# alv-around/mini-stark

Hardware: AMD Instinct MI355X
Metric: stark_proofs_per_s (higher is better)
Workload: dtype u64; 1 GPU; Fibonacci AIR, Goldilocks, 2^20 trace rows, blowup 8, 20 security bits (w=3, c=6, rounds=23, ood_queries=1, fri_queries=2); a step = 8 independent proofs in flight per GPU

## Files before the change

mini-stark_amd/csrc/fri_commit.cpp:

```cpp
#include "ctx.hpp"
#include "digest.hpp"
#include "fri_tail.hpp"

namespace msctx {

template <class F>
int Ctx<F>::round_commit(Round* r, size_t ncoef_in, int nonzero_limbs, const Round* prev, const XE* alpha) {
  if (ctz64(r->D) > F::TWO_ADICITY) return fail(MS_ERR_SHAPE, "FRI domain larger than the field's two-adicity");
  RQ(tree_shape(r->D, 2, 2, &r->ts));
  r->m = 0;
  r->base_cw = false;
  {
    const bool shard_next = shardable(r->D / 2);
    bool z_outside_base = false;
    for (int l = 1; l < E; l++) z_outside_base = z_outside_base || cur_z.c[l] != 0;
    if (prev && fri_pointwise && z_outside_base && prev->D == 2 * r->D && prev->ts.sharded == shard_next) {
      Plan* pl;
      RQ(get_plan(ctz64(prev->D), 0, false, &pl));
      const size_t W = (size_t)sh_world;
      const size_t m_out = shard_next ? r->D / (2 * W) : r->D;
      const size_t local = shard_next ? 2 * m_out : r->D;
      if (shard_next) r->m = m_out;
      if (r->cw.ensure(local * E * sizeof(T))) return fail(MS_ERR_NOMEM, "codeword");
      const size_t total = m_out * (shard_next ? 2 : 1);
// ... 239 lines not shown
  if (next_dist) { if (nr->poly.ensure(Sn * E * sizeof(T))) return fail(MS_ERR_NOMEM, "fold"); lq = nr->poly.template as<T>(); }
  else { if (d_lq.ensure(Sn * E * sizeof(T))) return fail(MS_ERR_NOMEM, "fold"); lq = d_lq.as<T>(); }
  if (d_folded.ensure((Sn + 1) * E * sizeof(T)) || d_carry.ensure(4096)) return fail(MS_ERR_NOMEM, "fold");
  if (4 * E * sizeof(T) * (size_t)sh_world > xcap) return fail(MS_ERR_NOMEM, "exchange buffers");
  size_t nq_coef = 0;
  PartScope part(this);
  if (m >= 2) {
    T* pay = reinterpret_cast<T*>(xs);
    typename mspoly::FoldKernel<F, E>::Params fp{lpoly(pr), lstride(pr), cntp, d_folded.as<T>(), Sn, a, pay};
    if (cnt) CK(run<mspoly::FoldKernel<F, E>>(K_FOLD, grid1(cnt, mspoly::THREADS), 1, mspoly::THREADS, 0, fp));
    else CK(msrt::memset_dev(xs, 0, 2 * E * sizeof(T), stream));
    const size_t mj = cnt ? cnt - 1 : 0;
    SHPlan pl; pl.nl = 0;
    if (mj) {
      if (d_sh.ensure(sh_scratch_elems(mj) * sizeof(T))) return fail(MS_ERR_NOMEM, "scan levels");
      pl = sh_plan(d_folded.as<T>(), Sn, 1, 1, mj, cur_z, lq, false, Sn, 1, 1, nullptr, d_sh.as<T>(), d_carry.as<T>(), pay + E, true);
      for (int l = 0; l + 1 < pl.nl; l++) RQ(sh_launch_inline(pl.agg[l], 0));
      RQ(sh_launch_inline(pl.top_agg, 0));
    }
    RQ(exchange(MS_XCHG_ALL_GATHER, 2 * E * sizeof(T)));
    typedef mspoly::ShardCarryKernel<F, E> CKn;
    typename CKn::Params cp;
    memset(&cp, 0, sizeof cp);
    cp.jobs = nullptr; cp.njobs = 1; cp.W = (u32)sh_world; cp.rank = (u32)sh_rank; cp.gathered = reinterpret_cast<const T*>(xr); cp.rank_stride = 2 * E;
    cp.inline_job.first_off = 0; cp.inline_job.agg_off = E; cp.inline_job.has_first = 1;
    cp.inline_job.zA = cur_z; cp.inline_job.zB = e_pow<F, E>(cur_z, (u64)(Sn - 1));
    cp.inline_job.scale = mj ? carry_scale(cur_z, mj, pl.P) : e_one<F, E>();
    cp.inline_job.carry_out = d_carry.as<T>();
    cp.inline_job.tail_out = cnt ? lq + (cnt - 1) : nullptr; cp.inline_job.tail_stride = Sn;
    cp.inline_job.h0_out = nullptr;
    CK(run<CKn>(K_SUFFIX_HORNER, 1, 1, CKn::THREADS, 0, cp));
    if (mj) for (int l = pl.nl - 1; l >= 0; l--) RQ(sh_launch_inline(pl.fin[l], 1));
    nq_coef = m - 1;
  }
  nr->S = Sn;
  if (next_dist) { nr->dist = true; nr->local_store = true; }
  else {
    if (nr->poly.ensure(nr->cap * E * sizeof(T))) return fail(MS_ERR_NOMEM, "fold");
    if (nq_coef) RQ(gather_poly(lq, Sn, nq_coef, nr->poly.template as<T>(), nr->cap));
    nr->S = 0;
  }
  *nq_coef_out = nq_coef;
  return 0;
}

template <class F>
int Ctx<F>::fri_tail_round(Round* pr, Round* nr, const XE& a, bool* done) {
  return msmerkle::with_digest(digest, [&](auto family) { return fri_tail_round_t<decltype(family)>(pr, nr, a, done); });
}
template <class F> template <class DG>
int Ctx<F>::fri_tail_round_t(Round* pr, Round* nr, const XE& a, bool* done) {
  *done = false;
  const size_t n = pr->ncoef, m = (n + 1) / 2, Dn = nr->D, M = Dn / 2;
  bool z_outside_base = false;
  for (int l = 1; l < E; l++) z_outside_base = z_outside_base || cur_z.c[l] != 0;
  if (!fri_tail_max || pr->D > fri_tail_max || pr->dist || pr->ts.sharded || shardable(M) || !fri_pointwise || !z_outside_base || m > (size_t)mspoly::SH_BS || M < 1) return 0;
  typedef msfri::FriTailKernel<F, E, DG> TK;
  if (M > (size_t)TK::WG_GROUPS << TK::TreeK::MAX_LEVELS) return 0;
  if (ctz64(Dn) > F::TWO_ADICITY) return fail(MS_ERR_SHAPE, "FRI domain larger than the field's two-adicity");
  RQ(tree_shape(Dn, 2, 2, &nr->ts));
  nr->m = 0; nr->base_cw = false;
  if (nr->poly.ensure(nr->cap * E * sizeof(T)) || d_folded.ensure((m + 1) * E * sizeof(T)) || nr->cw.ensure(Dn * E * sizeof(T)) || nr->nodes.ensure(nr->ts.nodes * 32) ||
      d_sh.ensure(sh_scratch_elems(m) * sizeof(T)))
    return fail(MS_ERR_NOMEM, "fused FRI round");
  Plan* pl;
  RQ(get_plan(ctz64(pr->D), 0, false, &pl));
  typename TK::Params tp;
  memset(&tp, 0, sizeof tp);
  tp.do_coef = m >= 2 ? 1 : 0;
  tp.fold = typename TK::FoldK::Params{pr->poly.template as<T>(), pr->cap, n, d_folded.as<T>(), m, a, nullptr};
  if (tp.do_coef) {
    SHPlan sp = sh_plan(d_folded.as<T>(), m, 0, 1, m, cur_z, nr->poly.template as<T>(), false, nr->cap, 0, 1, nullptr, d_sh.as<T>());
    if (sp.nl != 1) return fail(MS_ERR_STATE, "fused FRI round: scan of more than one block");
    tp.scan.jobs = nullptr; tp.scan.inline_job = sp.fin[0]; tp.scan.final_mode = 1;
  }
  tp.deg = typename TK::DegK::Params{nr->poly.template as<T>(), nr->cap, m >= 2 ? m - 1 : 0, res.word(Results::FRI_LEN), 0};
  const size_t per = M < (size_t)TK::WG_GROUPS ? M : (size_t)TK::WG_GROUPS, G = M / per;
  tp.G = (u32)G;
  const XE c = e_add<F, E>(cur_B[0], e_mul<F>(cur_B[1], a));
  tp.eval.src = pr->cw.template as<T>(); tp.eval.src_limb_stride = pr->D; tp.eval.dst = nr->cw.template as<T>(); tp.eval.dst_limb_stride = Dn;
  tp.eval.m_out = Dn; tp.eval.log_m = (u32)ctz64(Dn); tp.eval.groups = 1; tp.eval.shard_W = 0; tp.eval.shard_k = 0;
  tp.eval.tw_lo = pl->tw_lo.template as<T>(); tp.eval.tw_hi = pl->tw_hi.template as<T>(); tp.eval.lo_bits = (u32)pl->lo_bits; tp.eval.log_D = (u32)ctz64(pr->D);
  tp.eval.alpha = a; tp.eval.c2 = e_add<F, E>(c, c); tp.eval.z = cur_z; tp.eval.inv2 = f_inv<F>(F::from_u64(2));
  tp.leaf.base = nr->cw.template as<T>(); tp.leaf.col_stride = 0; tp.leaf.row_stride = 1; tp.leaf.limb_stride = Dn; tp.leaf.width = 1; tp.leaf.lpn = 2;
  tp.leaf.zero_as_empty = zae; tp.leaf.ngroups = M; tp.leaf.nodes = nr->nodes.template as<u32>();
  u32 nl = 0; while (((size_t)1 << nl) < per) nl++;
  tp.sub.nodes = nr->nodes.template as<u32>(); tp.sub.child_off = 0; tp.sub.nchildren = M; tp.sub.ic = 2; tp.sub.nlevels = nl;
  u32 tl = 0; while (((size_t)1 << tl) < G) tl++;
  tp.top.nodes = nr->nodes.template as<u32>(); tp.top.child_off = 2 * M - 2 * G; tp.top.nchildren = G; tp.top.ic = 2; tp.top.nlevels = tl;
  RQ(res.attach(tp.top));
  tp.root_index = nr->ts.nodes - 1;
  tp.done = reinterpret_cast<u32*>(res.word(Results::TAIL_DONE));
  next_bytes = (double)Dn * E * sizeof(T) * 3 + (double)M * 96;
  CK(run_coop<TK>(K_FRI_TAIL, (unsigned)(G + 1), TK::THREADS, TK::lds_bytes(), tp));
  *done = true;
  return 0;
}

template <class F>
int Ctx<F>::fri_fold_commit(const u64* alpha, u8* root) {
  if (!have_deep) return fail(MS_ERR_STATE, "fri_fold_commit before fri_deep");
  XE a;
  if (!alpha || !root || !load_ext(alpha, &a)) return fail(MS_ERR_ARG, "alpha");
  Round* pr = rounds[nrounds_done - 1];
  if (pr->D < 4) return fail(MS_ERR_SHAPE, "FRI round domain too small to fold (merkle.rs:93-104 panics)");
  const size_t n = pr->ncoef, m = (n + 1) / 2;
  Round* nr = round_slot(nrounds_done);
  nr->cap = m ? m : 1;
  nr->D = pr->D / 2;
  nr->dist = false; nr->local_store = false; nr->S = 0;
  size_t nq_coef = 0;
  bool fused = false, side = false;
  unsigned long long* dres = res.word(Results::FRI_LEN), ncoef = 0;
  auto stage = res.expect(dres, pr->dist && dist_chunk(nr->D) == pr->S / 2);
  RQ(fri_tail_round(pr, nr, a, &fused));
  if (!fused) {
  if (pr->dist) RQ(fold_dist(pr, nr, a, &nq_coef));
  else {
  if (nr->poly.ensure(nr->cap * E * sizeof(T)) || d_folded.ensure((m + 1) * E * sizeof(T))) return fail(MS_ERR_NOMEM, "fold");
  if (m >= 2) {
    side = fri_overlap && !prof_on;
    if (side) RQ(res.fork_side());
    StreamScope on_side(this, side ? side_stream : stream);
    typename mspoly::FoldKernel<F, E>::Params fp{pr->poly.template as<T>(), pr->cap, n, d_folded.as<T>(), m, a, nullptr};
    CK(run<mspoly::FoldKernel<F, E>>(K_FOLD, grid1(m, mspoly::THREADS), 1, mspoly::THREADS, 0, fp));
    RQ(suffix_horner(d_folded.as<T>(), m, 0, 1, m, cur_z, nr->poly.template as<T>(), nr->cap, 0, 1, nullptr));
    nq_coef = m - 1;
  }
  }
  if (nr->dist) {
    const size_t lc = lcount(nr, nq_coef);
    if (lc) {
      typename mspoly::DegreeKernel<F, E>::Params dp{lpoly(nr), lstride(nr), lc, dres, (size_t)sh_rank * nr->S};
      PartScope part(this);
      CK(run<mspoly::DegreeKernel<F, E>>(K_DEGREE, grid1(lc, mspoly::THREADS), 1, mspoly::THREADS, 0, dp));
    }
  } else if (nq_coef) {
    StreamScope on_side(this, side ? side_stream : stream);
    typename mspoly::DegreeKernel<F, E>::Params dp{nr->poly.template as<T>(), nr->cap, nq_coef, dres, 0};
    CK(run<mspoly::DegreeKernel<F, E>>(K_DEGREE, grid1(nq_coef, mspoly::THREADS), 1, mspoly::THREADS, 0, dp));
  }
  RQ(res.side_done());
  RQ(round_commit(nr, nq_coef, E, pr, &a));
  }
  RQ(read_root(nr->nodes, nr->ts, root, &ncoef));
  nr->ncoef = (size_t)ncoef;
  nrounds_done++; have_deep = false;
  return MS_OK;
}

template <class F>
int Ctx<F>::fri_round_info(int r, u64* ncoef, u64* D) {
  if (r < 0 || (size_t)r >= nrounds_done) return fail(MS_ERR_ARG, "round index");
  if (ncoef) *ncoef = rounds[r]->ncoef;
  if (D) *D = rounds[r]->D;
  return MS_OK;
}

template <class F>
int Ctx<F>::fri_round_poly_read(int r, u64* out) {
  if (r < 0 || (size_t)r >= nrounds_done || !out) return fail(MS_ERR_ARG, "round index");
  if (rounds[r]->local_store) return fail(MS_ERR_STATE, "round_poly_read: the polynomial of a sharded round is distributed over the ranks");
  return download_widen(rounds[r]->poly.template as<T>(), rounds[r]->ncoef, rounds[r]->cap, E, out);
}

template <class F>
int Ctx<F>::fri_round_codeword_read(int r, u64* out) {
// ... 28 lines not shown
```

mini-stark_amd/csrc/merkle.hpp:

```cpp
#pragma once
#include "field.hpp"

namespace msmerkle {

constexpr int THREADS = 256;
constexpr int OVF_WORDS = 2;
constexpr int OVF_LISTS = 256;
constexpr int PAD_GRID_Y = 4;
struct alignas(16) uint4_t { u32 x, y, z, w; };

MS_HD u32 rotr32(u32 x, int n) {
#if defined(__HIP_DEVICE_COMPILE__)
  return __builtin_amdgcn_alignbit(x, x, n);
#else
  return (x >> n) | (x << (32 - n));
#endif
}
MS_HD u32 bswap32(u32 x) { return __builtin_bswap32(x); }
MS_HD u32 ch3(u32 e, u32 f, u32 g) {
#if defined(__HIP_DEVICE_COMPILE__) && __has_builtin(__builtin_amdgcn_bitop3_b32)
  return __builtin_amdgcn_bitop3_b32(e, f, g, 0xCA);
#else
  return g ^ (e & (f ^ g));
#endif
}
MS_HD u32 maj3(u32 a, u32 b, u32 c) {
#if defined(__HIP_DEVICE_COMPILE__) && __has_builtin(__builtin_amdgcn_bitop3_b32)
  return __builtin_amdgcn_bitop3_b32(a, b, c, 0xE8);
#else
  return (a & b) | (c & (a | b));
#endif
}
MS_HD u32 xor3(u32 a, u32 b, u32 c) {
#if defined(__HIP_DEVICE_COMPILE__) && __has_builtin(__builtin_amdgcn_bitop3_b32)
  return __builtin_amdgcn_bitop3_b32(a, b, c, 0x96);
#else
  return a ^ b ^ c;
#endif
}

constexpr u32 SHA_K[64] = {
    0x428a2f98, 0x71374491, 0xb5c0fbcf, 0xe9b5dba5, 0x3956c25b, 0x59f111f1, 0x923f82a4, 0xab1c5ed5,
    0xd807aa98, 0x12835b01, 0x243185be, 0x550c7dc3, 0x72be5d74, 0x80deb1fe, 0x9bdc06a7, 0xc19bf174,
    0xe49b69c1, 0xefbe4786, 0x0fc19dc6, 0x240ca1cc, 0x2de92c6f, 0x4a7484aa, 0x5cb0a9dc, 0x76f988da,
    0x983e5152, 0xa831c66d, 0xb00327c8, 0xbf597fc7, 0xc6e00bf3, 0xd5a79147, 0x06ca6351, 0x14292967,
    0x27b70a85, 0x2e1b2138, 0x4d2c6dfc, 0x53380d13, 0x650a7354, 0x766a0abb, 0x81c2c92e, 0x92722c85,
    0xa2bfe8a1, 0xa81a664b, 0xc24b8b70, 0xc76c51a3, 0xd192e819, 0xd6990624, 0xf40e3585, 0x106aa070,
    0x19a4c116, 0x1e376c08, 0x2748774c, 0x34b0bcb5, 0x391c0cb3, 0x4ed8aa4a, 0x5b9cca4f, 0x682e6ff3,
    0x748f82ee, 0x78a5636f, 0x84c87814, 0x8cc70208, 0x90befffa, 0xa4506ceb, 0xbef9a3f7, 0xc67178f2};

struct PadBlockKW { u32 kw[64]; };
constexpr u32 c_rotr(u32 x, int n) { return (x >> n) | (x << (32 - n)); }
constexpr PadBlockKW make_pad_block_kw(u32 msg_bits) {
  PadBlockKW r{};
  u32 w[64] = {};
  w[0] = 0x80000000u; w[15] = msg_bits;
  for (int i = 16; i < 64; i++) {
    const u32 s0 = c_rotr(w[i - 15], 7) ^ c_rotr(w[i - 15], 18) ^ (w[i - 15] >> 3);
    const u32 s1 = c_rotr(w[i - 2], 17) ^ c_rotr(w[i - 2], 19) ^ (w[i - 2] >> 10);
    w[i] = w[i - 16] + s0 + w[i - 7] + s1;
  }
  for (int i = 0; i < 64; i++) r.kw[i] = SHA_K[i] + w[i];
  return r;
}
template <u32 MSG_BITS> struct PadBlock { static constexpr PadBlockKW T = make_pad_block_kw(MSG_BITS); };

struct Sha256 {
  u32 st[8];
  MS_HD void init() {
    st[0] = 0x6a09e667; st[1] = 0xbb67ae85; st[2] = 0x3c6ef372; st[3] = 0xa54ff53a;
    st[4] = 0x510e527f; st[5] = 0x9b05688c; st[6] = 0x1f83d9ab; st[7] = 0x5be0cd19;
  }
  MS_HD void compress(u32 (&w)[16]) {
    u32 a = st[0], b = st[1], c = st[2], d = st[3], e = st[4], f = st[5], g = st[6], h = st[7];
#pragma unroll
    for (int i = 0; i < 64; i++) {
      if (i >= 16) {
        u32 w15 = w[(i + 1) & 15], w2 = w[(i + 14) & 15];
        u32 s0 = xor3(rotr32(w15, 7), rotr32(w15, 18), w15 >> 3);
        u32 s1 = xor3(rotr32(w2, 17), rotr32(w2, 19), w2 >> 10);
        w[i & 15] = w[i & 15] + s0 + w[(i + 9) & 15] + s1;
      }
      u32 S1 = xor3(rotr32(e, 6), rotr32(e, 11), rotr32(e, 25));
      u32 ch = ch3(e, f, g);
      u32 t1 = h + S1 + ch + SHA_K[i] + w[i & 15];
      u32 S0 = xor3(rotr32(a, 2), rotr32(a, 13), rotr32(a, 22));
      u32 mj = maj3(a, b, c);
      u32 t2 = S0 + mj;
      h = g; g = f; f = e; e = d + t1; d = c; c = b; b = a; a = t1 + t2;
    }
    st[0] += a; st[1] += b; st[2] += c; st[3] += d; st[4] += e; st[5] += f; st[6] += g; st[7] += h;
  }
  template <u32 MSG_BITS> MS_HD void compress_pad_block() {
    u32 a = st[0], b = st[1], c = st[2], d = st[3], e = st[4], f = st[5], g = st[6], h = st[7];
#pragma unroll
    for (int i = 0; i < 64; i++) {
      u32 S1 = xor3(rotr32(e, 6), rotr32(e, 11), rotr32(e, 25));
      u32 ch = ch3(e, f, g);
      u32 t1 = h + S1 + ch + PadBlock<MSG_BITS>::T.kw[i];
      u32 S0 = xor3(rotr32(a, 2), rotr32(a, 13), rotr32(a, 22));
      u32 mj = maj3(a, b, c);
      u32 t2 = S0 + mj;
      h = g; g = f; f = e; e = d + t1; d = c; c = b; b = a; a = t1 + t2;
    }
    st[0] += a; st[1] += b; st[2] += c; st[3] += d; st[4] += e; st[5] += f; st[6] += g; st[7] += h;
  }
};

#ifndef MS_SUBTREE_PAIR_LEVELS
#define MS_SUBTREE_PAIR_LEVELS 1
#endif
struct Sha256Pair {
  u32 M, R1, R2, R3, Sa, Sb, Sc;
  bool a_lane;
  u32 cv[4];
  static MS_HD bool is_a_lane(int lane) { return (lane >> 2) & 1; }
  static MS_HD int node_in_group(int lane) { return is_a_lane(lane) ? 3 - (lane & 3) : (lane & 3); }
  MS_DEV void init(int lane) {
    a_lane = is_a_lane(lane);
    M = a_lane ? ~0u : 0u;
    R1 = a_lane ? 2 : 6; R2 = a_lane ? 13 : 11; R3 = a_lane ? 22 : 25;
    Sa = a_lane ? 17 : 7; Sb = a_lane ? 19 : 18; Sc = a_lane ? 10 : 3;
  }
  MS_DEV void reset() {
    cv[0] = a_lane ? 0x6a09e667u : 0x510e527fu; cv[1] = a_lane ? 0xbb67ae85u : 0x9b05688cu; cv[2] = a_lane ? 0x3c6ef372u : 0x1f83d9abu; cv[3] = a_lane ? 0xa54ff53au : 0x5be0cd19u;
  }
  MS_DEV void round(u32& x, u32& y, u32& z, u32& v, u32 kw) const {
    const u32 S = xor3(msrt::rotr_var(x, R1), msrt::rotr_var(x, R2), msrt::rotr_var(x, R3));
    const u32 xp = ms_bitop3<0x78>(x, z, M);
    const u32 F = ch3(xp, y, z);
    const u32 s = S + F;
    const u32 t = s + v + kw;
    const u32 n = msrt::pair_exchange_add(a_lane, v, t, s);
    v = z; z = y; y = x; x = n;
  }
  MS_DEV void compress(u32 (&w)[16]) {
    u32 x = cv[0], y = cv[1], z = cv[2], v = cv[3];
#pragma unroll
    for (int i = 0; i < 64; i++) {
      if (i >= 16) {
        const u32 r = ms_bitop3<0xE4>(w[(i + 14) & 15], w[(i + 1) & 15], M);
        const u32 o = ms_bitop3<0xE4>(w[(i + 9) & 15], w[i & 15], M);
        const u32 sig = xor3(msrt::rotr_var(r, Sa), msrt::rotr_var(r, Sb), r >> Sc);
        const u32 p = sig + o;
        w[i & 15] = p + msrt::pair_swap(p);
      }
      round(x, y, z, v, w[i & 15] + SHA_K[i]);
    }
    cv[0] += x; cv[1] += y; cv[2] += z; cv[3] += v;
  }
  template <u32 MSG_BITS> MS_DEV void compress_pad_block() {
    u32 x = cv[0], y = cv[1], z = cv[2], v = cv[3];
#pragma unroll
    for (int i = 0; i < 64; i++) round(x, y, z, v, PadBlock<MSG_BITS>::T.kw[i]);
    cv[0] += x; cv[1] += y; cv[2] += z; cv[3] += v;
  }
};

MS_HD u32 funnel_r(u32 hi, u32 lo, u32 sh) {
#if defined(__HIP_DEVICE_COMPILE__)
  return __builtin_amdgcn_alignbit(hi, lo, sh);
#else
  return sh ? ((hi << (32 - sh)) | (lo >> sh)) : lo;
#endif
}
MS_HD u32 drop_sel(u32 l) { return 0x07060504u - l * 0x01010101u; }
MS_HD u32 drop_bytes(u32 hi, u32 lo, u32 l, u32 sel) {
#if defined(__HIP_DEVICE_COMPILE__)
  (void)l;
  return __builtin_amdgcn_perm(hi, lo, sel);
#else
  (void)sel;
  return l ? ((hi << (8 * l)) | (lo >> (32 - 8 * l))) : hi;
#endif
}

template <int NWORDS, int NT> struct PackStream {
  u32* buf;
  u32 acc;
  u32 total;
  u32 done;
  u32 fbase;
  MS_HD void init_buf(u32* lds_words, int tid_) { buf = lds_words + tid_; acc = 0; total = 0; done = 0; fbase = 0; }
  template <int NW> MS_HD void append_words(const u32 (&W)[NW], u32 nbytes, u32 last4) {
    const u32 sh = 8u * (total & 3u);
    u32* wp = buf + ((total >> 2) - done) * NT;
    u32 prev = acc;
#pragma unroll
    for (int k = 0; k < NW; k++) { wp[k * NT] = funnel_r(prev, W[k], sh); prev = W[k]; }
    wp[NW * NT] = funnel_r(prev, 0u, sh);
    total += nbytes;
    acc = last4;
  }
  MS_HD void append_small(u32 w, u32 nbytes) {
    const u32 W[1] = {w};
    const u32 l4 = nbytes >= 4 ? w : ((acc << (8 * nbytes)) | (w >> (32 - 8 * nbytes)));
    append_words<1>(W, nbytes, l4);
  }
  MS_HD void begin_final() { fbase = done; }
};
template <int NWORDS, int NT, int MAXW, bool LAZY> struct ShaStream : PackStream<NWORDS, NT> {
  static_assert(NWORDS >= 16 + MAXW + 1 && NWORDS <= 48, "buffer = one or two blocks + room for one element");
  typedef PackStream<NWORDS, NT> Base;
  using Base::buf; using Base::total; using Base::done; using Base::fbase;
  Sha256 h;
  MS_HD void init(u32* lds_words, int tid_) { h.init(); Base::init_buf(lds_words, tid_); }
  MS_HD u32 end_message() { const u32 n = total; Base::append_small(0x80000000u, 1); Base::begin_final(); return n; }
  MS_HD void store_digest(u32* dst) const {
    uint4_t* out = reinterpret_cast<uint4_t*>(dst);
    uint4_t o0, o1;
    o0.x = bswap32(h.st[0]); o0.y = bswap32(h.st[1]); o0.z = bswap32(h.st[2]); o0.w = bswap32(h.st[3]);
    o1.x = bswap32(h.st[4]); o1.y = bswap32(h.st[5]); o1.z = bswap32(h.st[6]); o1.w = bswap32(h.st[7]);
    out[0] = o0; out[1] = o1;
  }
  enum { DONE = 0, MORE = 1, DEFER = 2 };
  MS_HD int drain(bool final, u32 msg_bytes) {
    if (!final) {
      const u32 pending = (total >> 2) - done;
      const bool go = LAZY ? msrt::wave_any(pending + (u32)MAXW + 1u > (u32)NWORDS) : true;
      if (go && pending >= 16) {
        u32 w[16];
#pragma unroll
        for (int i = 0; i < 16; i++) w[i] = buf[i * NT];
        h.compress(w);
        done += 16;
        u32 t[NWORDS - 16];
#pragma unroll
        for (int k = 0; k < NWORDS - 16; k++) t[k] = buf[(k + 16) * NT];
#pragma unroll
        for (int k = 0; k < NWORDS - 16; k++) buf[k * NT] = t[k];
      }
      return DONE;
    }
    const u32 valid_end = (total + 3) >> 2, limit = ((msg_bytes + 9 + 63) >> 6) << 4;
    if constexpr (!LAZY) {
      const u32 pending = limit - done;
      u32 w[16];
#pragma unroll
      for (int i = 0; i < 16; i++) w[i] = buf[i * NT];
#pragma unroll
      for (int i = 0; i < 16; i++) w[i] = (done + i < valid_end) ? w[i] : 0u;
      if (pending == 16) { w[14] = 0; w[15] = msg_bytes * 8u; }
      h.compress(w);
      done += 16;
      return pending == 32 ? DEFER : DONE;
    } else {
      const bool last = limit - done == 16;
      if (limit - 16 >= valid_end && last) return DEFER;
      u32 w[16];
      const u32* blk = buf + (done - fbase) * NT;
#pragma unroll
      for (int i = 0; i < 16; i++) w[i] = (done + i < valid_end) ? blk[i * NT] : 0u;
      if (last) { w[14] = 0; w[15] = msg_bytes * 8u; }
      h.compress(w);
      done += 16;
      if (limit == done) return DONE;
      return (limit - 16 >= valid_end && limit - done == 16) ? DEFER : MORE;
    }
  }
};

MS_HD u32 bcd4(u32 c) {
  const u32 q = (c * 5243u) >> 19;
  const u32 t = c + q * 65436u;
  const u32 tens = ((t * 103u) >> 10) & 0x000F000Fu;
  const u32 ones = t - tens * 10u;
  return (tens << 8) + ones;
}
MS_HD u32 pack4(u32 c) { return bcd4(c) + 0x30303030u; }
MS_HD u32 clz32(u32 x) { return (u32)__builtin_clz(x); }

MS_HD void dec_chunks(const GL&, u64 v, u32 (&c)[5]) {
  const u32 vh = (u32)(v >> 32);
  u32 q1 = (u32)(((u64)vh * 1934281311u) >> 32) >> 20;
  u64 r = v - (u64)q1 * 10000000000000000ULL;
  if (r >= 10000000000000000ULL) { r -= 10000000000000000ULL; q1++; }
  const u32 x = (u32)(r >> 22);
  u32 q2 = (u32)(((u64)x * 180143985u) >> 32);
  u32 r2 = (u32)r - q2 * 100000000u;
  if (r2 >= 100000000u) { r2 -= 100000000u; q2++; }
  c[0] = q1;
  c[1] = q2 / 10000u; c[2] = q2 - c[1] * 10000u;
  c[3] = r2 / 10000u; c[4] = r2 - c[3] * 10000u;
}
MS_HD void dec_chunks(const BB&, u64 v, u32 (&c)[3]) {
  const u32 x = (u32)v;
  c[0] = x / 100000000u; const u32 r = x - c[0] * 100000000u;
  c[1] = r / 10000u; c[2] = r - c[1] * 10000u;
}

template <class F, class S> MS_HD void put_dec(S& s, typename F::T v_, int zero_as_empty) {
  const u64 v = F::to_u64(v_);
  constexpr int NCH = (F::MAX_DIGITS + 3) / 4;
  u32 c[NCH];
  dec_chunks(F(), v, c);
  if (c[0] != 0) {
    u32 W[NCH];
    const u32 b0 = bcd4(c[0]);
    const u32 lead = clz32(b0) >> 3;
    W[0] = b0 + 0x30303030u;
#pragma unroll
    for (int j = 1; j < NCH; j++) W[j] = pack4(c[j]);
    const u32 sel = drop_sel(lead);
    u32 X[NCH];
#pragma unroll
    for (int j = 0; j + 1 < NCH; j++) X[j] = drop_bytes(W[j], W[j + 1], lead, sel);
    X[NCH - 1] = drop_bytes(W[NCH - 1], 0u, lead, sel);
    s.template append_words<NCH>(X, 4u * NCH - lead, W[NCH - 1]);
    return;
  }
  if (v == 0) { if (!zero_as_empty) s.append_small(0x30000000u, 1); return; }
  u32 lead = 0; bool found = false;
#pragma unroll
  for (int j = 0; j < NCH; j++) {
    const u32 z = c[j] == 0 ? 4u : (c[j] < 10u ? 3u : (c[j] < 100u ? 2u : (c[j] < 1000u ? 1u : 0u)));
    if (!found) lead += z;
    found = found || (c[j] != 0);
  }
  for (int j = 1; j < NCH; j++) {
    const int k = 4 * (j + 1) - (int)lead;
    if (k >= 4) s.append_small(pack4(c[j]), 4);
    else if (k > 0) s.append_small(pack4(c[j]) << (8 * (4 - k)), (u32)k);
  }
}
template <int E> struct Affix;
template <> struct Affix<1> {
  static constexpr int MAX_BYTES = 0;
  template <class S> static MS_HD void before(S&, u32) {}
  template <class S> static MS_HD void after(S&, u32) {}
};
template <class S> MS_HD void put_open(S& s) { const u32 W[4] = {0x51756164u, 0x45787446u, 0x69656c64u, 0x28000000u}; s.template append_words<4>(W, 13, 0x656c6428u); }
template <class S> MS_HD void put_plus(S& s) { s.append_small(0x202b2000u, 3); }
template <class S> MS_HD void put_close(S& s) { const u32 W[2] = {0x202a2075u, 0x29000000u}; s.template append_words<2>(W, 5, 0x2a207529u); }
template <> struct Affix<2> {
  static constexpr int MAX_BYTES = 13;
  template <class S> static MS_HD void before(S& s, u32 k) { if (k == 0) put_open(s); else put_plus(s); }
  template <class S> static MS_HD void after(S& s, u32 k) { if (k == 1) put_close(s); }
};
template <> struct Affix<4> {
  static constexpr int MAX_BYTES = 26;
  template <class S> static MS_HD void before(S& s, u32 k) {
    if (k == 0) {
      const u32 W[7] = {0x51756164u, 0x45787446u, 0x69656c64u, 0x28517561u, 0x64457874u, 0x4669656cu, 0x64280000u};
      s.template append_words<7>(W, 26, 0x656c6428u);
    } else if (k == 2) {
      const u32 W[4] = {0x202b2051u, 0x75616445u, 0x78744669u, 0x656c6428u};
      s.template append_words<4>(W, 16, 0x656c6428u);
    } else put_plus(s);
  }
  template <class S> static MS_HD void after(S& s, u32 k) {
    if (k == 1) put_close(s);
    else if (k == 3) {
      const u32 W[3] = {0x202a2075u, 0x29202a20u, 0x75290000u};
      s.template append_words<3>(W, 10, 0x2a207529u);
    }
  }
};

constexpr int LIN_MAXT = 4;
struct LinColSpec { u32 n ; u32 src[LIN_MAXT]; u64 s[LIN_MAXT]; };
struct Sha256Kernels;
template <class F, int E, bool LAZY = false, class DG = Sha256Kernels> struct LeafHashKernel {
  typedef typename F::T T;
  static constexpr int THREADS = msmerkle::THREADS;
  struct Params {
    const T* base; size_t col_stride, row_stride, limb_stride;
    u32 width, lpn; int zero_as_empty;
    size_t ngroups;
    u32* nodes;
    u32* ovf_count; u32* ovf; u32 ovf_cap;
    size_t g_first; u32 run_len, run_stride;
    const LinColSpec* lin;
    size_t out_g0;
  };
  static constexpr int MAX_BYTES = F::MAX_DIGITS + Affix<E>::MAX_BYTES;
  static constexpr int MAXW = (3 + MAX_BYTES + 3) / 4 + 1;
  static constexpr int NWORDS = DG::BLOCK_WORDS * (LAZY ? DG::LAZY_BLOCKS : 1) + MAXW + 1 + DG::EXTRA_WORDS;
  typedef typename DG::template Stream<NWORDS, THREADS, MAXW, LAZY> Stream;
  static MS_HD int nphases(const Params&) { return 1; }
  static MS_HD size_t lds_bytes() { return (size_t)NWORDS * THREADS * sizeof(u32); }
  static MS_DEV void phase(int, const Params& p, int bx, int, int tid, int nthreads, unsigned char* lds) {
    size_t g = (size_t)bx * nthreads + tid;
    if (g >= p.ngroups) return;
    if (p.run_len) g = p.g_first + (g / p.run_len) * (size_t)p.run_stride + g % p.run_len;
    Stream s; s.init(reinterpret_cast<u32*>(lds), tid);
    size_t f = g * p.lpn;
    size_t row = f / p.width; u32 col = (u32)(f - row * p.width);
    const u32 nlimbs = p.lpn * (u32)E;
    u32 msg_bytes = 0;
    bool deferred = false;
    for (u32 j = 0; LAZY || j <= nlimbs; j++) {
      if (j < nlimbs) {
        const u32 k = j & (u32)(E - 1);
        const T* rowp = p.base + row * p.row_stride + (size_t)k * p.limb_stride;
        T v;
        if (p.lin && p.lin[col].n) {
          const LinColSpec& lc = p.lin[col];
          v = 0;
          for (u32 t = 0; t < lc.n; t++) {
            const T x = rowp[(size_t)lc.src[t] * p.col_stride];
            if (lc.s[t] == 1) v = F::add(v, x);
            else if (lc.s[t] == F::P - 1) v = F::sub(v, x);
            else v = F::add(v, F::mul(x, F::from_u64(lc.s[t])));
          }
        } else v = rowp[(size_t)col * p.col_stride];
        Affix<E>::before(s, k);
        put_dec<F>(s, v, p.zero_as_empty);
        Affix<E>::after(s, k);
        if (k == (u32)(E - 1) && ++col == p.width) { col = 0; row++; }
      } else if (j == nlimbs) {
        msg_bytes = s.end_message();
      }
      const int st = s.drain(j >= nlimbs, msg_bytes);
      if constexpr (LAZY) { if (j >= nlimbs && st != Stream::MORE) { deferred = st == Stream::DEFER; break; } }
      else deferred = st == Stream::DEFER;
    }
    if constexpr (!DG::DEFERS) { s.store_digest(p.nodes + (g - p.out_g0) * 8); }
    else {
      if (deferred && !p.ovf) {
        u32 w[16];
#pragma unroll
        for (int i = 0; i < 15; i++) w[i] = 0;
        w[15] = msg_bytes * 8u;
        s.h.compress(w);
        deferred = false;
      }
      const u32 list = (u32)bx % (u32)OVF_LISTS;
      const u32 slot = msrt::wave_alloc_slot(p.ovf_count + list, deferred);
      const size_t go = g - p.out_g0;
      if (deferred) {
        u32* e = p.ovf + ((size_t)list * p.ovf_cap + slot) * OVF_WORDS;
        e[0] = (u32)go; e[1] = msg_bytes * 8u;
        u32* st = p.nodes + go * 8;
#pragma unroll
        for (int i = 0; i < 8; i++) st[i] = s.h.st[i];
        return;
      }
      s.store_digest(p.nodes + go * 8);
    }
  }
};
struct PadOnlyBlockKernel {
  static constexpr int THREADS = msmerkle::THREADS;
  struct Params { const u32* ovf_count; const u32* ovf; u32 ovf_cap; u32* nodes; };
  static MS_HD int nphases(const Params&) { return 1; }
  static MS_DEV void phase(int, const Params& p, int bx, int by, int tid, int nthreads, unsigned char*) {
    const u32 n = p.ovf_count[bx];
    const u32 stride = (u32)nthreads * PAD_GRID_Y;
    for (u32 t = (u32)by * nthreads + tid; t < n; t += stride) {
      const u32* e = p.ovf + ((size_t)bx * p.ovf_cap + t) * OVF_WORDS;
      Sha256 h;
      const u32* st = p.nodes + (size_t)e[0] * 8;
#pragma unroll
      for (int i = 0; i < 8; i++) h.st[i] = st[i];
      u32 w[16];
#pragma unroll
      for (int i = 0; i < 15; i++) w[i] = 0;
      w[15] = e[1];
      h.compress(w);
      uint4_t* out = reinterpret_cast<uint4_t*>(p.nodes + (size_t)e[0] * 8);
      uint4_t o0, o1;
      o0.x = bswap32(h.st[0]); o0.y = bswap32(h.st[1]); o0.z = bswap32(h.st[2]); o0.w = bswap32(h.st[3]);
      o1.x = bswap32(h.st[4]); o1.y = bswap32(h.st[5]); o1.z = bswap32(h.st[6]); o1.w = bswap32(h.st[7]);
      out[0] = o0; out[1] = o1;
    }
  }
};

struct InnerHashParams { u32* nodes; size_t child_off, nchildren; u32 ic; u32 nlevels; u32* host_root;
                         unsigned long long* aux_src; unsigned long long* aux_dst;
                         msrt::HostFlag flag;  };
template <int IC> struct InnerHashKernelT {
  static constexpr int THREADS = msmerkle::THREADS;
  typedef InnerHashParams Params;
  static MS_HD int nphases(const Params& p) { return (int)p.nlevels; }
  static MS_DEV void phase(int ph, const Params& p, int bx, int, int tid, int nthreads, unsigned char*) {
    const u32 ic = IC ? (u32)IC : p.ic;
    size_t child_off = p.child_off, nchildren = p.nchildren;
    for (int l = 0; l < ph; l++) { child_off += nchildren; nchildren /= ic; }
    const size_t nparents = nchildren / ic;
    const size_t stride = (p.nlevels > 1) ? (size_t)nthreads : 0;
    for (size_t g = (size_t)bx * nthreads + tid; g < nparents; g += stride) {
      const u32* ch = p.nodes + (child_off + g * ic) * 8;
      Sha256 h; h.init();
      u32 w[16];
      for (u32 b = 0; b < ic / 2; b++) {
        const uint4_t* c4 = reinterpret_cast<const uint4_t*>(ch + b * 16);
#pragma unroll
        for (int q = 0; q < 4; q++) {
          const uint4_t v = c4[q];
          w[4 * q] = bswap32(v.x); w[4 * q + 1] = bswap32(v.y); w[4 * q + 2] = bswap32(v.z); w[4 * q + 3] = bswap32(v.w);
        }
        h.compress(w);
      }
      if constexpr (IC > 0) h.template compress_pad_block<(u32)IC * 256u>();
      else {
        w[0] = 0x80000000u;
#pragma unroll
        for (int i = 1; i < 15; i++) w[i] = 0;
        w[15] = ic * 256u;
        h.compress(w);
      }
      uint4_t* out = reinterpret_cast<uint4_t*>(p.nodes + (child_off + nchildren + g) * 8);
      uint4_t o0, o1;
      o0.x = bswap32(h.st[0]); o0.y = bswap32(h.st[1]); o0.z = bswap32(h.st[2]); o0.w = bswap32(h.st[3]);
      o1.x = bswap32(h.st[4]); o1.y = bswap32(h.st[5]); o1.z = bswap32(h.st[6]); o1.w = bswap32(h.st[7]);
      out[0] = o0; out[1] = o1;
      if (p.host_root && nparents == 1) {
        uint4_t* hr = reinterpret_cast<uint4_t*>(p.host_root); hr[0] = o0; hr[1] = o1;
        if (p.aux_src) { *p.aux_dst = *p.aux_src; *p.aux_src = 0; }
        msrt::raise_host_flag(p.flag);
      }
      if (stride == 0) break;
    }
  }
};

typedef InnerHashKernelT<0> InnerHashKernel;
typedef InnerHashKernelT<2> InnerHashKernel2;

struct InnerSubtreeKernel {
  static constexpr int THREADS = msmerkle::THREADS;
  static constexpr int MAX_LEVELS = 9;
  static_assert((1 << (MAX_LEVELS - 1)) == THREADS, "level 0 of a workgroup: one parent per thread");
  typedef InnerHashParams Params;
  static MS_HD size_t lds_bytes() { return (size_t)(THREADS + THREADS / 2) * 32; }
  static MS_DEV void run(const Params& p, int bx, int, int, int tid, unsigned char* lds) {
    u32* const buf0 = reinterpret_cast<u32*>(lds);
    u32* const buf1 = buf0 + (size_t)THREADS * 8;
    const u32 nl = p.nlevels;
    size_t child_off = p.child_off, nchildren = p.nchildren;
    u32 pp = 1u << nl;
    Sha256Pair hp; hp.init(tid);
    for (u32 l = 0; l < nl; l++) {
      pp >>= 1;
      const size_t nparents = nchildren >> 1;
      if (MS_SUBTREE_PAIR_LEVELS && 2 * pp <= (u32)THREADS) {
        const u32 nact = 2 * pp < 8 ? 8 : 2 * pp;
        if ((u32)tid < nact) {
          const u32 nd0 = ((u32)tid >> 3) * 4 + (u32)Sha256Pair::node_in_group(tid);
          const bool live = nd0 < pp;
          const u32 nd = live ? nd0 : 0;
// ... 296 lines not shown
```

mini-stark_amd/csrc/merkle_tree.cpp:

```cpp
#include "ctx.hpp"
#include "digest.hpp"
#include "grind.hpp"

namespace msctx {

template <class F>
int Ctx<F>::tree_shape(size_t leaf_num, size_t lpn, size_t ic, TreeShape* ts) {
  if (lpn == 0 || ic < 2 || !is_pow2(ic)) return fail(MS_ERR_SHAPE, "merkle: bad leafs_per_node / inner_children");
  const size_t node_num = leaf_num / lpn;
  long lg = log_two_k(node_num, ic);
  if (lg < 0) return fail(MS_ERR_SHAPE, lg == -1 ? "number if not a power of 2" : "number if not a power of base");
  if (leaf_num % lpn != 0) return fail(MS_ERR_SHAPE, "merkle: leaf_num % leafs_per_node != 0");
  if (lg >= 64 || node_num == 0) return fail(MS_ERR_SHAPE, "Tree is not full!");
  ts->leaf_num = leaf_num; ts->lpn = lpn; ts->ic = ic; ts->levels = (size_t)lg + 1;
  size_t total = 0, m = node_num;
  for (;;) { total += m; if (m == 1) break; m /= ic; }
  ts->nodes = total; ts->local_nodes = total; ts->Mloc = 0; ts->sharded = false;
  return 0;
}

template <class F> template <int EL>
int Ctx<F>::leaf_hash(const T* base, size_t col_stride, size_t row_stride, size_t limb_stride, u32 width, size_t lpn, size_t ngroups, u32* out,
              size_t g_first, u32 run_len, u32 run_stride, const msmerkle::LinColSpec* lin, size_t out_g0) {
  if (ngroups >> 32) return fail(MS_ERR_SHAPE, "more than 2^32 leaf groups");
  const size_t nwg = grid1(ngroups, msmerkle::THREADS);
  auto launch = [&](auto kernel, u32* counters, size_t cap) -> int {
    typedef decltype(kernel) LK;
    typename LK::Params lp;
    lp.base = base; lp.col_stride = col_stride; lp.row_stride = row_stride; lp.limb_stride = limb_stride;
    lp.width = width; lp.lpn = (u32)lpn; lp.zero_as_empty = zae; lp.ngroups = ngroups; lp.nodes = out;
    lp.ovf_count = counters; lp.ovf = counters ? d_ovf.as<u32>() : nullptr; lp.ovf_cap = (u32)cap;
    lp.g_first = g_first; lp.run_len = run_len; lp.run_stride = run_stride; lp.lin = lin; lp.out_g0 = out_g0;
    next_bytes = (double)ngroups * (lpn * EL * sizeof(T) + 32);
    CK(run<LK>(K_LEAF_HASH, (unsigned)nwg, 1, msmerkle::THREADS, LK::lds_bytes(), lp));
    return 0;
  };
  auto hash = [&](auto family) -> int {
    typedef decltype(family) DG;
    const size_t lists = msmerkle::OVF_LISTS, cap = DG::DEFERS ? ((nwg + lists - 1) / lists) * msmerkle::THREADS : 0;
    void* counters = nullptr;
    if constexpr (DG::DEFERS) {
      if (d_ovf.ensure(lists * cap * msmerkle::OVF_WORDS * 4)) return fail(MS_ERR_NOMEM, "deferred-block lists");
      RQ(zero_alloc(lists * 4, &counters));
    }
    if (lpn * EL >= (size_t)leaf_lazy_min) RQ(launch(msmerkle::LeafHashKernel<F, EL, true, DG>(), reinterpret_cast<u32*>(counters), cap));
    else RQ(launch(msmerkle::LeafHashKernel<F, EL, false, DG>(), reinterpret_cast<u32*>(counters), cap));
    if constexpr (DG::DEFERS) {
      msmerkle::PadOnlyBlockKernel::Params pp{reinterpret_cast<u32*>(counters), d_ovf.as<u32>(), (u32)cap, out};
      const size_t used = nwg < lists ? nwg : lists, per_list = grid1(cap, msmerkle::THREADS);
      CK(run<msmerkle::PadOnlyBlockKernel>(K_LEAF_HASH, (unsigned)used, (unsigned)(per_list < (size_t)msmerkle::PAD_GRID_Y ? per_list : (size_t)msmerkle::PAD_GRID_Y), msmerkle::THREADS, 0, pp));
    }
    return 0;
  };
  return msmerkle::with_digest(digest, [&](auto family) -> int {
    typedef decltype(family) DG;
    if constexpr (std::is_same<DG, msmerkle::Blake3Kernels>::value) {
      const size_t bound = lpn * EL * (size_t)msmerkle::LeafHashKernel<F, EL, false, DG>::MAX_BYTES;
      if (lpn > DG::MAX_BYTES || bound > DG::MAX_BYTES)
        return fail(MS_ERR_ARG, "BLAKE3: a leaf group's message may exceed 16384 bytes (leafs_per_node x limbs x longest decimal): not supported by the BLAKE3 kernels");
      if (bound > DG::CHUNK_BYTES) return hash(typename DG::Multi());
    }
    return hash(family);
  });
}

template <class F> template <int EL>
int Ctx<F>::tree_build(const T* base, size_t col_stride, size_t row_stride, size_t limb_stride, u32 width, const TreeShape& ts, DevBuf& nodes, const msmerkle::LinColSpec* lin) {
  if (nodes.ensure(ts.nodes * 32)) return fail(MS_ERR_NOMEM, "merkle nodes");
  const size_t ngroups = ts.leaf_num / ts.lpn;
  RQ((leaf_hash<EL>(base, col_stride, row_stride, limb_stride, width, ts.lpn, ngroups, nodes.as<u32>(), 0, 0, 0, lin)));
  RQ(inner_levels(nodes.as<u32>(), ngroups, ts.ic));
  return 0;
}

template <class F>
int Ctx<F>::inner_launch(unsigned grid, const msmerkle::InnerHashParams& ip) {
  return msmerkle::with_digest(digest, [&](auto family) -> int {
    typedef decltype(family) DG;
    if constexpr (std::is_same<DG, msmerkle::Blake3Kernels>::value) {
      if (ip.ic > DG::MAX_BYTES / 32) return fail(MS_ERR_ARG, "BLAKE3: inner nodes of more than 512 children (16384 bytes) are not supported by the BLAKE3 kernels");
      if (ip.ic > DG::CHUNK_BYTES / 32) {
        CK(run<typename DG::InnerMulti>(K_INNER_HASH, grid, 1, msmerkle::THREADS, DG::InnerMulti::lds_bytes(), ip));
        return 0;
      }
    }
    if (ip.ic == 2) CK(run<typename DG::Inner2>(K_INNER_HASH, grid, 1, msmerkle::THREADS, 0, ip));
    else CK(run<typename DG::Inner>(K_INNER_HASH, grid, 1, msmerkle::THREADS, 0, ip));
    return 0;
  });
}

template <class F>
int Ctx<F>::inner_levels(u32* nodes, size_t nchildren, size_t ic, bool final_levels, u8* rec_out) {
  size_t child_off = 0;
  unsigned long long* const shard_aux = res.shard_word();
  bool rec_done = false;
  auto to_rec = [&](msmerkle::InnerHashKernel::Params& ip) {
    ip.host_root = reinterpret_cast<u32*>(rec_out);
    if (shard_aux) { ip.aux_src = shard_aux; ip.aux_dst = reinterpret_cast<unsigned long long*>(rec_out + 32); }
    rec_done = true;
  };
  while (nchildren > 1) {
    msmerkle::InnerHashKernel::Params ip;
    ip.nodes = nodes; ip.child_off = child_off; ip.nchildren = nchildren; ip.ic = (u32)ic; ip.host_root = nullptr; ip.aux_src = nullptr; ip.aux_dst = nullptr; ip.flag = msrt::HostFlag{nullptr, 0};
    const size_t nparents = nchildren / ic;
    if (ic == 2 && nparents <= subtree_parents && (nchildren & (nchildren - 1)) == 0) {
      typedef msmerkle::InnerSubtreeKernel SK;
      u32 nl = 0; for (size_t m = nchildren; m > 1 && nl < (u32)SK::MAX_LEVELS; m >>= 1) nl++;
      const size_t left = nchildren >> nl;
      if (final_levels && left == 1) RQ(res.attach(ip));
      else if (rec_out && left == 1) to_rec(ip);
      ip.nlevels = nl;
      next_bytes = (double)nchildren * 32 * 2;
      CK(msmerkle::with_digest(digest, [&](auto family) { return run_coop<typename decltype(family)::Subtree>(K_INNER_HASH, (unsigned)left, SK::THREADS, SK::lds_bytes(), ip); }));
      for (u32 l = 0; l < nl; l++) { child_off += nchildren; nchildren >>= 1; }
      continue;
    }
    if (final_levels && (nparents == 1 || nparents <= (size_t)tree_top_parents)) RQ(res.attach(ip));
    else if (rec_out && (nparents == 1 || nparents <= (size_t)tree_top_parents)) to_rec(ip);
    if (nparents <= (size_t)tree_top_parents) {
      u32 nl = 0; for (size_t m = nchildren; m > 1; m /= ic) nl++;
      ip.nlevels = nl;
      next_bytes = (double)nchildren * 32 * 2;
      RQ(inner_launch(1, ip));
      break;
    }
    ip.nlevels = 1;
    next_bytes = (double)nparents * (ic * 32 + 32);
    RQ(inner_launch((unsigned)((nparents + msmerkle::THREADS - 1) / msmerkle::THREADS), ip));
    child_off += nchildren; nchildren = nparents;
  }
  if (rec_out && !rec_done) {
    CK(msrt::d2d(rec_out, reinterpret_cast<u8*>(nodes) + (child_off + nchildren - 1) * 32, 32, stream));
// ... 145 lines not shown
```

Before: 281.4 proofs/s.

## Streamline SHA-256 leaf hashing and precompute pad-only block schedules

Three changes to the SHA-256 Merkle leaf path. The leaf kernel now walks the input with a pointer that advances by fixed steps instead of recomputing a row and column address for every limb, using a template flag for groups that span whole rows. The non-lazy stream zeroes its buffer up front so the per-word mask before compression can be dropped. The pad-only deferred block kernel gains a first phase that builds message-schedule-plus-constant tables in LDS for up to eight nearby length values, so most deferred blocks skip the message expansion. The costs are an extra phase, some LDS use, branch divergence between table and fallback paths, and twice as many kernel instantiations.

Result: no change. 284.0 proofs/s (median of 6 runs) (+0.9%).

```diff
diff --git a/mini-stark_amd/csrc/fri_commit.cpp b/mini-stark_amd/csrc/fri_commit.cpp
--- a/mini-stark_amd/csrc/fri_commit.cpp
+++ b/mini-stark_amd/csrc/fri_commit.cpp
@@ -345,7 +345,7 @@
   tp.eval.m_out = Dn; tp.eval.log_m = (u32)ctz64(Dn); tp.eval.groups = 1; tp.eval.shard_W = 0; tp.eval.shard_k = 0;
   tp.eval.tw_lo = pl->tw_lo.template as<T>(); tp.eval.tw_hi = pl->tw_hi.template as<T>(); tp.eval.lo_bits = (u32)pl->lo_bits; tp.eval.log_D = (u32)ctz64(pr->D);
   tp.eval.alpha = a; tp.eval.c2 = e_add<F, E>(c, c); tp.eval.z = cur_z; tp.eval.inv2 = f_inv<F>(F::from_u64(2));
-  tp.leaf.base = nr->cw.template as<T>(); tp.leaf.col_stride = 0; tp.leaf.row_stride = 1; tp.leaf.limb_stride = Dn; tp.leaf.width = 1; tp.leaf.lpn = 2;
+  tp.leaf.base = nr->cw.template as<T>(); tp.leaf.col_stride = 0; tp.leaf.row_stride = 1; tp.leaf.limb_stride = Dn; tp.leaf.width = 1; tp.leaf.lpn = 2; tp.leaf.rows_per_group = 2;
   tp.leaf.zero_as_empty = zae; tp.leaf.ngroups = M; tp.leaf.nodes = nr->nodes.template as<u32>();
   u32 nl = 0; while (((size_t)1 << nl) < per) nl++;
   tp.sub.nodes = nr->nodes.template as<u32>(); tp.sub.child_off = 0; tp.sub.nchildren = M; tp.sub.ic = 2; tp.sub.nlevels = nl;
diff --git a/mini-stark_amd/csrc/merkle.hpp b/mini-stark_amd/csrc/merkle.hpp
--- a/mini-stark_amd/csrc/merkle.hpp
+++ b/mini-stark_amd/csrc/merkle.hpp
@@ -64,6 +64,22 @@
   return r;
 }
 template <u32 MSG_BITS> struct PadBlock { static constexpr PadBlockKW T = make_pad_block_kw(MSG_BITS); };
+template <int STRIDE> MS_HD void pad_only_block_kw(u32 msg_bits, u32* dst) {
+  u32 w[16];
+#pragma unroll
+  for (int i = 0; i < 15; i++) w[i] = 0;
+  w[15] = msg_bits;
+#pragma unroll
+  for (int i = 0; i < 64; i++) {
+    if (i >= 16) {
+      const u32 w15 = w[(i + 1) & 15], w2 = w[(i + 14) & 15];
+      const u32 s0 = c_rotr(w15, 7) ^ c_rotr(w15, 18) ^ (w15 >> 3);
+      const u32 s1 = c_rotr(w2, 17) ^ c_rotr(w2, 19) ^ (w2 >> 10);
+      w[i & 15] = w[i & 15] + s0 + w[(i + 9) & 15] + s1;
+    }
+    dst[i * STRIDE] = SHA_K[i] + w[i & 15];
+  }
+}
 
 struct Sha256 {
   u32 st[8];
@@ -98,6 +114,20 @@
       u32 S1 = xor3(rotr32(e, 6), rotr32(e, 11), rotr32(e, 25));
       u32 ch = ch3(e, f, g);
       u32 t1 = h + S1 + ch + PadBlock<MSG_BITS>::T.kw[i];
+      u32 S0 = xor3(rotr32(a, 2), rotr32(a, 13), rotr32(a, 22));
+      u32 mj = maj3(a, b, c);
+      u32 t2 = S0 + mj;
+      h = g; g = f; f = e; e = d + t1; d = c; c = b; b = a; a = t1 + t2;
+    }
+    st[0] += a; st[1] += b; st[2] += c; st[3] += d; st[4] += e; st[5] += f; st[6] += g; st[7] += h;
+  }
+  template <int STRIDE> MS_HD void compress_kw(const u32* kw) {
+    u32 a = st[0], b = st[1], c = st[2], d = st[3], e = st[4], f = st[5], g = st[6], h = st[7];
+#pragma unroll
+    for (int i = 0; i < 64; i++) {
+      u32 S1 = xor3(rotr32(e, 6), rotr32(e, 11), rotr32(e, 25));
+      u32 ch = ch3(e, f, g);
+      u32 t1 = h + S1 + ch + kw[i * STRIDE];
       u32 S0 = xor3(rotr32(a, 2), rotr32(a, 13), rotr32(a, 22));
       u32 mj = maj3(a, b, c);
       u32 t2 = S0 + mj;
@@ -204,7 +234,13 @@
   typedef PackStream<NWORDS, NT> Base;
   using Base::buf; using Base::total; using Base::done; using Base::fbase;
   Sha256 h;
-  MS_HD void init(u32* lds_words, int tid_) { h.init(); Base::init_buf(lds_words, tid_); }
+  MS_HD void init(u32* lds_words, int tid_) {
+    h.init(); Base::init_buf(lds_words, tid_);
+    if constexpr (!LAZY) {
+#pragma unroll
+      for (int k = 0; k < NWORDS; k++) buf[k * NT] = 0u;
+    }
+  }
   MS_HD u32 end_message() { const u32 n = total; Base::append_small(0x80000000u, 1); Base::begin_final(); return n; }
   MS_HD void store_digest(u32* dst) const {
     uint4_t* out = reinterpret_cast<uint4_t*>(dst);
@@ -229,6 +265,10 @@
         for (int k = 0; k < NWORDS - 16; k++) t[k] = buf[(k + 16) * NT];
 #pragma unroll
         for (int k = 0; k < NWORDS - 16; k++) buf[k * NT] = t[k];
+        if constexpr (!LAZY) {
+#pragma unroll
+          for (int k = NWORDS - 16; k < NWORDS; k++) buf[k * NT] = 0u;
+        }
       }
       return DONE;
     }
@@ -238,8 +278,6 @@
       u32 w[16];
 #pragma unroll
       for (int i = 0; i < 16; i++) w[i] = buf[i * NT];
-#pragma unroll
-      for (int i = 0; i < 16; i++) w[i] = (done + i < valid_end) ? w[i] : 0u;
       if (pending == 16) { w[14] = 0; w[15] = msg_bytes * 8u; }
       h.compress(w);
       done += 16;
@@ -360,7 +398,7 @@
 constexpr int LIN_MAXT = 4;
 struct LinColSpec { u32 n ; u32 src[LIN_MAXT]; u64 s[LIN_MAXT]; };
 struct Sha256Kernels;
-template <class F, int E, bool LAZY = false, class DG = Sha256Kernels> struct LeafHashKernel {
+template <class F, int E, bool LAZY = false, class DG = Sha256Kernels, bool ANYW = false> struct LeafHashKernel {
   typedef typename F::T T;
   static constexpr int THREADS = msmerkle::THREADS;
   struct Params {
@@ -372,6 +410,7 @@
     size_t g_first; u32 run_len, run_stride;
     const LinColSpec* lin;
     size_t out_g0;
+    u32 rows_per_group;
   };
   static constexpr int MAX_BYTES = F::MAX_DIGITS + Affix<E>::MAX_BYTES;
   static constexpr int MAXW = (3 + MAX_BYTES + 3) / 4 + 1;
@@ -384,18 +423,22 @@
     if (g >= p.ngroups) return;
     if (p.run_len) g = p.g_first + (g / p.run_len) * (size_t)p.run_stride + g % p.run_len;
     Stream s; s.init(reinterpret_cast<u32*>(lds), tid);
-    size_t f = g * p.lpn;
-    size_t row = f / p.width; u32 col = (u32)(f - row * p.width);
+    size_t row; u32 col;
+    if constexpr (ANYW) { const size_t f = g * p.lpn; row = f / p.width; col = (u32)(f - row * p.width); }
+    else { row = g * p.rows_per_group; col = 0; }
+    const T* lp = p.base + row * p.row_stride + (size_t)col * p.col_stride;
+    const size_t elem_step = p.col_stride - (size_t)(E - 1) * p.limb_stride;
+    const size_t wrap_step = elem_step + p.row_stride - (size_t)p.width * p.col_stride;
     const u32 nlimbs = p.lpn * (u32)E;
     u32 msg_bytes = 0;
     bool deferred = false;
     for (u32 j = 0; LAZY || j <= nlimbs; j++) {
       if (j < nlimbs) {
         const u32 k = j & (u32)(E - 1);
-        const T* rowp = p.base + row * p.row_stride + (size_t)k * p.limb_stride;
         T v;
         if (p.lin && p.lin[col].n) {
           const LinColSpec& lc = p.lin[col];
+          const T* rowp = lp - (size_t)col * p.col_stride;
           v = 0;
           for (u32 t = 0; t < lc.n; t++) {
             const T x = rowp[(size_t)lc.src[t] * p.col_stride];
@@ -403,11 +446,15 @@
             else if (lc.s[t] == F::P - 1) v = F::sub(v, x);
             else v = F::add(v, F::mul(x, F::from_u64(lc.s[t])));
           }
-        } else v = rowp[(size_t)col * p.col_stride];
+        } else v = *lp;
         Affix<E>::before(s, k);
         put_dec<F>(s, v, p.zero_as_empty);
         Affix<E>::after(s, k);
-        if (k == (u32)(E - 1) && ++col == p.width) { col = 0; row++; }
+        if (k == (u32)(E - 1)) {
+          const bool wrap = ++col == p.width;
+          if (wrap) col = 0;
+          lp += (ptrdiff_t)(wrap ? wrap_step : elem_step);
+        } else lp += (ptrdiff_t)p.limb_stride;
       } else if (j == nlimbs) {
         msg_bytes = s.end_message();
       }
@@ -443,21 +490,37 @@
 struct PadOnlyBlockKernel {
   static constexpr int THREADS = msmerkle::THREADS;
   struct Params { const u32* ovf_count; const u32* ovf; u32 ovf_cap; u32* nodes; };
-  static MS_HD int nphases(const Params&) { return 1; }
-  static MS_DEV void phase(int, const Params& p, int bx, int by, int tid, int nthreads, unsigned char*) {
+  static constexpr int TAB_ROWS = 8;
+  static MS_HD int nphases(const Params&) { return 2; }
+  static MS_HD size_t lds_bytes() { return (size_t)64 * TAB_ROWS * sizeof(u32); }
+  static MS_DEV void phase(int ph, const Params& p, int bx, int by, int tid, int nthreads, unsigned char* lds) {
     const u32 n = p.ovf_count[bx];
+    const u32 first = (u32)by * nthreads;
+    if (first >= n) return;
+    const u32* list = p.ovf + (size_t)bx * p.ovf_cap * OVF_WORDS;
+    u32* tab = reinterpret_cast<u32*>(lds);
+    const u32 bits0 = (list[(size_t)first * OVF_WORDS + 1] & ~511u) + 448u;
+    const bool tables = n - first > 64u;
+    if (ph == 0) {
+      if (tables && tid < TAB_ROWS) pad_only_block_kw<TAB_ROWS>(bits0 + 8u * (u32)tid, tab + tid);
+      return;
+    }
     const u32 stride = (u32)nthreads * PAD_GRID_Y;
-    for (u32 t = (u32)by * nthreads + tid; t < n; t += stride) {
-      const u32* e = p.ovf + ((size_t)bx * p.ovf_cap + t) * OVF_WORDS;
+    for (u32 t = first + tid; t < n; t += stride) {
+      const u32* e = list + (size_t)t * OVF_WORDS;
       Sha256 h;
       const u32* st = p.nodes + (size_t)e[0] * 8;
 #pragma unroll
       for (int i = 0; i < 8; i++) h.st[i] = st[i];
-      u32 w[16];
-#pragma unroll
-      for (int i = 0; i < 15; i++) w[i] = 0;
-      w[15] = e[1];
-      h.compress(w);
+      const u32 row = (e[1] - bits0) >> 3;
+      if (tables && row < (u32)TAB_ROWS) h.template compress_kw<TAB_ROWS>(tab + row);
+      else {
+        u32 w[16];
+#pragma unroll
+        for (int i = 0; i < 15; i++) w[i] = 0;
+        w[15] = e[1];
+        h.compress(w);
+      }
       uint4_t* out = reinterpret_cast<uint4_t*>(p.nodes + (size_t)e[0] * 8);
       uint4_t o0, o1;
       o0.x = bswap32(h.st[0]); o0.y = bswap32(h.st[1]); o0.z = bswap32(h.st[2]); o0.w = bswap32(h.st[3]);
diff --git a/mini-stark_amd/csrc/merkle_tree.cpp b/mini-stark_amd/csrc/merkle_tree.cpp
--- a/mini-stark_amd/csrc/merkle_tree.cpp
+++ b/mini-stark_amd/csrc/merkle_tree.cpp
@@ -31,6 +31,7 @@
     lp.width = width; lp.lpn = (u32)lpn; lp.zero_as_empty = zae; lp.ngroups = ngroups; lp.nodes = out;
     lp.ovf_count = counters; lp.ovf = counters ? d_ovf.as<u32>() : nullptr; lp.ovf_cap = (u32)cap;
     lp.g_first = g_first; lp.run_len = run_len; lp.run_stride = run_stride; lp.lin = lin; lp.out_g0 = out_g0;
+    lp.rows_per_group = (u32)(lpn / width);
     next_bytes = (double)ngroups * (lpn * EL * sizeof(T) + 32);
     CK(run<LK>(K_LEAF_HASH, (unsigned)nwg, 1, msmerkle::THREADS, LK::lds_bytes(), lp));
     return 0;
@@ -43,12 +44,15 @@
       if (d_ovf.ensure(lists * cap * msmerkle::OVF_WORDS * 4)) return fail(MS_ERR_NOMEM, "deferred-block lists");
       RQ(zero_alloc(lists * 4, &counters));
     }
-    if (lpn * EL >= (size_t)leaf_lazy_min) RQ(launch(msmerkle::LeafHashKernel<F, EL, true, DG>(), reinterpret_cast<u32*>(counters), cap));
-    else RQ(launch(msmerkle::LeafHashKernel<F, EL, false, DG>(), reinterpret_cast<u32*>(counters), cap));
+    const bool lazy = lpn * EL >= (size_t)leaf_lazy_min, whole_rows = lpn % width == 0;
+    if (lazy && whole_rows) RQ(launch(msmerkle::LeafHashKernel<F, EL, true, DG>(), reinterpret_cast<u32*>(counters), cap));
+    else if (lazy) RQ(launch(msmerkle::LeafHashKernel<F, EL, true, DG, true>(), reinterpret_cast<u32*>(counters), cap));
+    else if (whole_rows) RQ(launch(msmerkle::LeafHashKernel<F, EL, false, DG>(), reinterpret_cast<u32*>(counters), cap));
+    else RQ(launch(msmerkle::LeafHashKernel<F, EL, false, DG, true>(), reinterpret_cast<u32*>(counters), cap));
     if constexpr (DG::DEFERS) {
       msmerkle::PadOnlyBlockKernel::Params pp{reinterpret_cast<u32*>(counters), d_ovf.as<u32>(), (u32)cap, out};
       const size_t used = nwg < lists ? nwg : lists, per_list = grid1(cap, msmerkle::THREADS);
-      CK(run<msmerkle::PadOnlyBlockKernel>(K_LEAF_HASH, (unsigned)used, (unsigned)(per_list < (size_t)msmerkle::PAD_GRID_Y ? per_list : (size_t)msmerkle::PAD_GRID_Y), msmerkle::THREADS, 0, pp));
+      CK(run<msmerkle::PadOnlyBlockKernel>(K_LEAF_HASH, (unsigned)used, (unsigned)(per_list < (size_t)msmerkle::PAD_GRID_Y ? per_list : (size_t)msmerkle::PAD_GRID_Y), msmerkle::THREADS, msmerkle::PadOnlyBlockKernel::lds_bytes(), pp));
     }
     return 0;
   };
```
